# cyanreg/ffmpeg_ffv2

Hardware: AMD Instinct MI355X
Metric: Mpix/s encode (4K yuv420p10, slices=8) at 1/2/4/8 GPUs; bit-exact vs CPU (higher is better)
Workload: dtype int32

## Files before the change

### ffmpeg_ffv2_amd/csrc/ffv2_capi.cpp

```cpp
#include "../../include/ffv2_amd.h"
#include "ffv2_kernels.h"

#include <float.h>
#include <math.h>
#include <stdio.h>
#include <stdlib.h>
#include <string.h>

#include <atomic>
#include <chrono>
#include <condition_variable>
#include <functional>
#include <mutex>
#include <thread>
#include <vector>

#include "gen/scan_lut.h"

#define FFV2AMD_VERSION "ffv2-amd 0.1 (gfx950)"

namespace {

inline uint32_t coded_gain_host(int64_t e)
{
// ... 496 lines not shown
    }
    return FFV2AMD_ERR_INVAL;
}

size_t align_up(size_t v, size_t a) { return (v + a - 1) / a * a; }

}

struct ffv2amd_encoder;
static void lanecoder_free(ffv2amd_encoder *e);

struct ffv2amd_encoder {
    ffv2amd_info info{};
    FFV2Geom geom{};
    int device = 0;
    hipStream_t stream = nullptr;
    int64_t  *d_thr = nullptr;
    uint16_t *d_lds_scan = nullptr;
    uint8_t  *d_prefix = nullptr;
    int prefix_len = 0, slack = 0;
    uint32_t *d_codes = nullptr, *d_bitoff = nullptr;
    int32_t  *d_status = nullptr;
    int32_t  *d_err = nullptr;
    uint8_t  *d_frame = nullptr, *d_pkt = nullptr;
    uint32_t *d_meta = nullptr;
    int32_t  *d_w1 = nullptr;
    uint8_t  *h_frame = nullptr, *h_pkt = nullptr;
    uint32_t *h_meta = nullptr;
    int32_t *d_coef_ws = nullptr;
    int16_t *d_y = nullptr, *h_y = nullptr;
    uint32_t *h_codes = nullptr;
    uint8_t *d_pk_ws = nullptr;
    int32_t *d_inv_plane = nullptr;
    uint32_t *d_sizes_ws = nullptr;
    int32_t *coef_sink = nullptr;
    int profiling = 0;
    unsigned prof_calls = 0;
    struct EvTriple { hipEvent_t a, b, c, d; bool d_is_b; };
    bool pipelined = false;
    hipStream_t e_stream = nullptr;
    hipEvent_t evT[2] = { nullptr, nullptr }, evE[2] = { nullptr, nullptr };
    bool evE_valid[2] = { false, false };
    uint32_t *d_codes2 = nullptr, *d_bitoff2 = nullptr;
    int32_t *d_status2 = nullptr;
    unsigned seq = 0;
    int seq_pb = 0;
// ... 22 lines not shown
    bool device_coder = false;
    QpSet qset[2];
    size_t q_stream_stride = 0;
    hipStream_t q_copy = nullptr;
    unsigned q_sub = 0, q_fin = 0;
    uint8_t *qh_frame[2] = { nullptr, nullptr }, *qd_frame[2] = { nullptr, nullptr };
    int32_t *qd_w[2] = { nullptr, nullptr };
    uint8_t *qd_c420[2] = { nullptr, nullptr };
    int64_t q_tag[2] = { 0, 0 };
    int16_t *d_dec_pulses = nullptr;
    float *d_dec_mag = nullptr;
    int32_t *d_dec_c0 = nullptr, *d_dec_coef = nullptr;
    uint8_t *d_dec_frame = nullptr;
    int32_t *d_wide_plane = nullptr, *d_wide_c0 = nullptr;
    int64_t *d_wide_en = nullptr;
    FFV2Upconv *upconv = nullptr;
    bool upconv_tried = false;
    uint8_t *d_420 = nullptr, *h_420 = nullptr;
    struct RingSlot {
        uint8_t  *h_frame = nullptr, *d_frame = nullptr;
        uint8_t  *d_pkt = nullptr, *h_pkt = nullptr;
        uint32_t *d_meta = nullptr, *h_meta = nullptr;
        uint32_t *d_codes = nullptr, *d_bitcnt = nullptr;
        int32_t  *d_w = nullptr;
        bool has_w = false;
        uint8_t  *d_c420 = nullptr;
        hipEvent_t ev_h2d = nullptr, ev_done = nullptr, ev_meta = nullptr;
        int64_t tag = 0;
    };
    std::vector<RingSlot> ring;
    int ring_head = 0, ring_count = 0;
    hipStream_t ring_h2d = nullptr, ring_comp[2] = { nullptr, nullptr }, ring_d2h = nullptr, ring_pkt = nullptr;
    GatherPool *ring_pool = nullptr;
    unsigned ring_seq = 0;
    struct RegRange { const uint8_t *base; size_t bytes; };
    std::vector<RegRange> ring_reg;
    struct LaneCoder {
        int cap = 0;
        int group = 0;
        int32_t *d_coef = nullptr;
        int16_t *d_y = nullptr;
        uint32_t *d_bitcnt = nullptr;
        FFV2LaneCoderArgs a{};
        uint2 *d_split = nullptr;
        struct Set {
            uint32_t *d_codes = nullptr, *bits = nullptr, *rowbase = nullptr, *gbase = nullptr, *rawbase = nullptr, *delta = nullptr;
// ... 64 lines not shown

#define HIPCHK(x) do { hipError_t e_ = (x); if (e_ != hipSuccess) { \
    fprintf(stderr, "ffv2amd: %s failed: %s\n", #x, hipGetErrorString(e_)); \
    (void)hipGetLastError();       \
    return FFV2AMD_ERR_DEVICE; } } while (0)

struct DeviceGuard {
    int prev = -1;
    bool ok = false;
    explicit DeviceGuard(int dev)
    {
        if (hipGetDevice(&prev) != hipSuccess) prev = -1;
        ok = (prev == dev) || hipSetDevice(dev) == hipSuccess;
        if (prev == dev) prev = -1;
    }
    ~DeviceGuard() { if (prev >= 0) (void)hipSetDevice(prev); }
};

extern "C" void ffv2amd_ring_close(ffv2amd_encoder *e);
static int encode_uploaded_frame(ffv2amd_encoder *e, int qp, const int32_t *W, uint8_t *out, size_t out_cap, size_t *out_size);

static int launch_encode_qp0(ffv2amd_encoder *e, int nframes, const void *d_frames, const int32_t *d_W,
                             void *d_packets, size_t packet_stride, uint32_t *d_sizes, int32_t *status,
                             uint32_t *codes, uint32_t *bitcnt, int32_t *coef, hipStream_t st, hipStream_t se,
                             ffv2amd_encoder::EvTriple *ev, int32_t *err)
{
    FFV2TStageArgs a{};
    a.g = e->geom; a.nframes = nframes; a.frames = (const uint8_t *)d_frames;
    a.coef = coef; a.energy = nullptr; a.codes = codes; a.bitcnt = bitcnt; a.W = d_W;
    a.gain_thr = e->d_thr; a.gain_n = GAIN_TABLE_N; a.lds_scan = e->d_lds_scan;
    a.status = err;
    a.zero = (uint32_t *)d_packets; a.zero_stride_dw = (uint32_t)(packet_stride / 4);
    if (ev) HIPCHK(hipEventRecord(ev->a, st));
    HIPCHK(ffv2_launch_tstage(a, st));
    if (ev) HIPCHK(hipEventRecord(ev->b, st));
    if (se != st) {
        hipEvent_t join = e->evT[e->seq_pb];
        HIPCHK(hipEventRecord(join, st));
        HIPCHK(hipStreamWaitEvent(se, join, 0));
    }
    if (ev && se != st) HIPCHK(hipEventRecord(ev->d, se));
    if (ev) ev->d_is_b = se == st;
    FFV2EStageArgs b{};
    b.g = e->geom; b.nframes = nframes; b.codes = codes; b.bitoff = bitcnt;
    b.packets = (uint8_t *)d_packets; b.packet_stride = packet_stride;
    b.sizes = d_sizes; b.status = status; b.err = err;
    b.prefix = e->d_prefix; b.prefix_len = e->prefix_len; b.slack_bits = e->slack;
    b.header_bits = ((uint32_t)e->info.pix_fmt & 15u) | (1u << 4);
    b.header_nbits = 5;
    HIPCHK(ffv2_launch_estage_qp0(b, se));
    if (ev) HIPCHK(hipEventRecord(ev->c, se));
    return FFV2AMD_OK;
}

extern "C" {

const char *ffv2amd_version(void) { return FFV2AMD_VERSION; }

uint32_t ffv2amd_coded_gain(int64_t energy) { return coded_gain_host(energy); }

int ffv2amd_range_prefix(int pix_fmt, int num_sb, uint8_t *out, size_t cap, int *slack_bits)
{
    std::vector<uint8_t> b;
    int sl = 0;
    int r = range_prefix(pix_fmt, num_sb, b, &sl);
    if (r < 0) return r;
    if (b.size() > cap) return FFV2AMD_ERR_NOSPACE;
// ... 13 lines not shown
    (void)hipFree(e->d_420);
    if (e->h_420) (void)hipHostFree(e->h_420);
    lanecoder_free(e);
    for (auto &q : e->qset) {
        (void)hipFree(q.d_rec); (void)hipFree(q.d_stream); (void)hipFree(q.d_totals); (void)hipFree(q.d_codes); (void)hipFree(q.d_status);
        if (q.h_rec) (void)hipHostFree(q.h_rec);
        if (q.h_stream) (void)hipHostFree(q.h_stream);
        if (q.h_totals) (void)hipHostFree(q.h_totals);
        if (q.h_codes) (void)hipHostFree(q.h_codes);
        if (q.h_status) (void)hipHostFree(q.h_status);
        if (q.ev) (void)hipEventDestroy(q.ev);
        for (auto ev : q.ev_frame) if (ev) (void)hipEventDestroy(ev);
        (void)hipFree(q.d_pre); (void)hipFree(q.d_raw); (void)hipFree(q.d_pk); (void)hipFree(q.d_pk_sizes); (void)hipFree(q.d_pk_status);
        if (q.h_pk_sizes) (void)hipHostFree(q.h_pk_sizes);
        if (q.h_pk_status) (void)hipHostFree(q.h_pk_status);
    }
    if (e->q_copy) { (void)hipStreamSynchronize(e->q_copy); (void)hipStreamDestroy(e->q_copy); }
    for (int k = 0; k < 2; k++) {
        (void)hipFree(e->qd_frame[k]); (void)hipFree(e->qd_w[k]); (void)hipFree(e->qd_c420[k]);
        if (e->qh_frame[k]) (void)hipHostFree(e->qh_frame[k]);
    }
    (void)hipFree(e->d_thr); (void)hipFree(e->d_lds_scan); (void)hipFree(e->d_prefix);
    (void)hipFree(e->d_codes); (void)hipFree(e->d_bitoff); (void)hipFree(e->d_status); (void)hipFree(e->d_err);
    (void)hipFree(e->d_frame); (void)hipFree(e->d_pkt); (void)hipFree(e->d_meta); (void)hipFree(e->d_w1);
    (void)hipFree(e->d_inv_plane);
    (void)hipFree(e->d_wide_plane); (void)hipFree(e->d_wide_c0); (void)hipFree(e->d_wide_en);
    (void)hipFree(e->d_dec_pulses); (void)hipFree(e->d_dec_mag); (void)hipFree(e->d_dec_c0); (void)hipFree(e->d_dec_coef);
    (void)hipFree(e->d_dec_frame);
    (void)hipFree(e->d_coef_ws); (void)hipFree(e->d_y); (void)hipFree(e->d_pk_ws); (void)hipFree(e->d_sizes_ws);
    if (e->h_y) (void)hipHostFree(e->h_y);
    if (e->h_codes) (void)hipHostFree(e->h_codes);
    if (e->h_frame) (void)hipHostFree(e->h_frame);
    if (e->h_pkt) (void)hipHostFree(e->h_pkt);
    if (e->h_meta) (void)hipHostFree(e->h_meta);
    for (auto &t : e->ev_pool) { (void)hipEventDestroy(t.a); (void)hipEventDestroy(t.b); (void)hipEventDestroy(t.c); (void)hipEventDestroy(t.d); }
    if (e->e_stream) { (void)hipStreamSynchronize(e->e_stream); (void)hipStreamDestroy(e->e_stream); }
    for (int i = 0; i < 2; i++) { if (e->evT[i]) (void)hipEventDestroy(e->evT[i]); if (e->evE[i]) (void)hipEventDestroy(e->evE[i]); }
    (void)hipFree(e->d_codes2); (void)hipFree(e->d_bitoff2); (void)hipFree(e->d_status2);
    if (e->stream) (void)hipStreamDestroy(e->stream);
    (void)hipGetLastError();
    delete e;
}

int ffv2amd_encoder_create(ffv2amd_encoder **out, int width, int height, int pix_fmt,
                           int device, int max_batch)
{
// ... 41 lines not shown
    g.width = width; g.height = height; g.depth = depth; g.planes = planes; g.bytes_per_sample = bps;
    g.nsx = in.num_sb_x; g.nsy = in.num_sb_y; g.nblk = in.block_planes;
    g.row_pitch = in.row_pitch; g.plane_stride = in.plane_stride; g.frame_stride = in.frame_stride;
    g.inv_planes = (uint32_t)(((uint64_t)1 << 32) / (uint32_t)planes + 1);
    g.inv_nsx = (uint32_t)(((uint64_t)1 << 32) / (uint32_t)g.nsx + 1);

    std::call_once(g_thr_once, build_gain_table);
    uint16_t lds_scan[4096];
    for (int i = 0; i < 8; i++)
        for (int l = 0; l < 64; l++)
            for (int e = 0; e < 8; e++) {
                const int q = 256 * (2 * i + e / 4) + 4 * l + (e & 3);
                lds_scan[(i * 64 + l) * 8 + e] =
                    (uint16_t)(((FFV2_SCAN_LUT[q] >> 6) * 69 + (FFV2_SCAN_LUT[q] & 63)) * 4);
            }

#define CK(x) do { if ((x) != hipSuccess) { fprintf(stderr, "ffv2amd: %s failed: %s\n", #x, hipGetErrorString(hipGetLastError())); \
    ffv2amd_encoder_destroy(e); return FFV2AMD_ERR_DEVICE; } } while (0)
    CK(hipStreamCreateWithFlags(&e->stream, hipStreamNonBlocking));
    CK(hipMalloc(&e->d_thr, sizeof(int64_t) * GAIN_TABLE_N));
    CK(hipMemcpy(e->d_thr, g_thr.data(), sizeof(int64_t) * GAIN_TABLE_N, hipMemcpyHostToDevice));
    CK(hipMalloc(&e->d_lds_scan, sizeof(lds_scan)));
    CK(hipMemcpy(e->d_lds_scan, lds_scan, sizeof(lds_scan), hipMemcpyHostToDevice));
    CK(hipMalloc(&e->d_prefix, align_up(prefix.size(), 16)));
    CK(hipMemcpy(e->d_prefix, prefix.data(), prefix.size(), hipMemcpyHostToDevice));
    CK(hipMalloc(&e->d_codes, sizeof(uint32_t) * FFV2_CODES_PER_BP * g.nblk * (size_t)max_batch));
    CK(hipMalloc(&e->d_bitoff, sizeof(uint32_t) * g.nblk * (size_t)max_batch));
    CK(hipMalloc(&e->d_status, sizeof(int32_t) * (size_t)max_batch));
    CK(hipMalloc(&e->d_err, sizeof(int32_t) * 2 * (size_t)max_batch));
    CK(hipMemsetAsync(e->d_err, 0, sizeof(int32_t) * 2 * (size_t)max_batch, e->stream));
    CK(hipStreamSynchronize(e->stream));
    CK(hipStreamSynchronize(nullptr));
    CK(hipMalloc(&e->d_frame, in.frame_stride));
    CK(hipMalloc(&e->d_pkt, in.packet_cap));
    CK(hipMalloc(&e->d_meta, 16));
    CK(hipMalloc(&e->d_w1, sizeof(int32_t) * g.nblk));
    CK(hipHostMalloc(&e->h_frame, in.frame_stride, hipHostMallocDefault));
    CK(hipHostMalloc(&e->h_pkt, in.packet_cap, hipHostMallocDefault));
    CK(hipHostMalloc(&e->h_meta, 16, hipHostMallocDefault));
#undef CK
    memset(e->h_frame, 0, in.frame_stride);
    *out = e;
    return FFV2AMD_OK;
}

int ffv2amd_encoder_info(const ffv2amd_encoder *e, ffv2amd_info *info)
{
    if (!e || !info) return FFV2AMD_ERR_INVAL;
    *info = e->info;
    return FFV2AMD_OK;
}

int ffv2amd_tstage_device(ffv2amd_encoder *e, int nframes, const void *d_frames,
// ... 30 lines not shown
    const int pb = pipe ? (int)(e->seq++ & 1u) : 0;
    int32_t *status = d_status ? d_status : (pb ? e->d_status2 : e->d_status);
    uint32_t *codes = pb ? e->d_codes2 : e->d_codes, *bitcnt = pb ? e->d_bitoff2 : e->d_bitoff;
    hipStream_t se = pipe ? e->e_stream : s;
    if (pipe && e->evE_valid[pb])
        HIPCHK(hipStreamWaitEvent(s, e->evE[pb], 0));
    ffv2amd_encoder::EvTriple *ev = nullptr;
    if (e->profiling > 0 && (e->prof_calls++ % (unsigned)e->profiling) == 0) {
        if (e->ev_used == e->ev_pool.size()) {
            if (e->ev_pool.size() >= 8192) {
                double t, x, lo, hi; int n;
                ffv2amd_profile_read_ex(e, &t, &x, &n, &lo, &hi);
                e->prof_t = t; e->prof_e = x; e->prof_n = n; e->prof_tmin = lo; e->prof_tmax = hi;
            } else {
                ffv2amd_encoder::EvTriple t{};
                HIPCHK(hipEventCreate(&t.a)); HIPCHK(hipEventCreate(&t.b)); HIPCHK(hipEventCreate(&t.c));
                HIPCHK(hipEventCreate(&t.d));
                try { e->ev_pool.push_back(t); } catch (...) { return FFV2AMD_ERR_NOMEM; }
            }
        }
        ev = &e->ev_pool[e->ev_used++];
    }
    e->seq_pb = pb;
    int r = launch_encode_qp0(e, nframes, d_frames, d_W, d_packets, packet_stride, d_sizes, status, codes, bitcnt,
                              e->coef_sink, s, se, ev, e->d_err + (size_t)pb * e->info.max_batch);
    if (r < 0) return r;
    if (pipe) {
        HIPCHK(hipEventRecord(e->evE[pb], se));
        e->evE_valid[pb] = true;
    }
    return FFV2AMD_OK;
}

int ffv2amd_encoder_set_pipelined(ffv2amd_encoder *e, int on)
{
    if (!e) return FFV2AMD_ERR_INVAL;
    DeviceGuard guard(e->device);
    if (!guard.ok) return FFV2AMD_ERR_DEVICE;
    if (on && !e->e_stream) {
        const size_t nb = (size_t)e->info.block_planes, B = (size_t)e->info.max_batch;
        HIPCHK(hipStreamCreateWithFlags(&e->e_stream, hipStreamNonBlocking));
        for (int i = 0; i < 2; i++) {
            HIPCHK(hipEventCreateWithFlags(&e->evT[i], hipEventDisableTiming));
            HIPCHK(hipEventCreateWithFlags(&e->evE[i], hipEventDisableTiming));
        }
        HIPCHK(hipMalloc(&e->d_codes2, sizeof(uint32_t) * FFV2_CODES_PER_BP * nb * B));
        HIPCHK(hipMalloc(&e->d_bitoff2, sizeof(uint32_t) * nb * B));
        HIPCHK(hipMalloc(&e->d_status2, sizeof(int32_t) * B));
// ... 1518 lines not shown
                                     h_packets + (size_t)f * packet_stride, packet_stride, &n);
        } catch (...) { r = FFV2AMD_ERR_NOMEM; }
        h_status[f] = r;
        h_sizes[f] = r < 0 ? 0 : (uint32_t)n;
    });
    if (trace) {
        const auto t_end = std::chrono::steady_clock::now();
        fprintf(stderr, "ffv2amd: qp=%d batch of %d: device (T-stage + PVQ + copies) %.3f ms, host range coder %.3f ms\n",
                qp, nframes, std::chrono::duration<double, std::milli>(t_dev - t_begin).count(),
                std::chrono::duration<double, std::milli>(t_end - t_dev).count());
    }
    return FFV2AMD_OK;
}


void ffv2amd_ring_close(ffv2amd_encoder *e)
{
    if (!e || e->ring.empty()) return;
    (void)hipSetDevice(e->device);
    for (hipStream_t st : { e->ring_h2d, e->ring_comp[0], e->ring_comp[1], e->ring_d2h, e->ring_pkt })
        if (st) (void)hipStreamSynchronize(st);
    for (auto &r : e->ring) {
        (void)hipFree(r.d_frame); (void)hipFree(r.d_pkt); (void)hipFree(r.d_meta);
        (void)hipFree(r.d_codes); (void)hipFree(r.d_bitcnt); (void)hipFree(r.d_w); (void)hipFree(r.d_c420);
        if (r.h_frame) (void)hipHostFree(r.h_frame);
        if (r.h_pkt) (void)hipHostFree(r.h_pkt);
        if (r.h_meta) (void)hipHostFree(r.h_meta);
        if (r.ev_h2d) (void)hipEventDestroy(r.ev_h2d);
        if (r.ev_done) (void)hipEventDestroy(r.ev_done);
        if (r.ev_meta) (void)hipEventDestroy(r.ev_meta);
    }
    e->ring.clear();
    for (auto &g : e->ring_reg) (void)hipHostUnregister((void *)g.base);
    e->ring_reg.clear();
    if (e->ring_pool) { e->ring_pool->shutdown(); delete e->ring_pool; e->ring_pool = nullptr; }
    for (hipStream_t *st : { &e->ring_h2d, &e->ring_comp[0], &e->ring_comp[1], &e->ring_d2h, &e->ring_pkt })
        if (*st) { (void)hipStreamDestroy(*st); *st = nullptr; }
    e->ring_head = e->ring_count = 0;
}

int ffv2amd_ring_open(ffv2amd_encoder *e, int depth)
{
    if (!e || depth < 1 || depth > 64) return FFV2AMD_ERR_INVAL;
    if (!e->ring.empty()) return FFV2AMD_ERR_INVAL;
    DeviceGuard guard(e->device);
    if (!guard.ok) return FFV2AMD_ERR_DEVICE;
    const ffv2amd_info &in = e->info;
    const size_t nb = (size_t)in.block_planes;
#define RK(x) do { if ((x) != hipSuccess) { fprintf(stderr, "ffv2amd: %s failed: %s\n", #x, hipGetErrorString(hipGetLastError())); \
    ffv2amd_ring_close(e); return FFV2AMD_ERR_DEVICE; } } while (0)
    try { e->ring.resize((size_t)depth); } catch (...) { return FFV2AMD_ERR_NOMEM; }
    RK(hipStreamCreateWithFlags(&e->ring_h2d, hipStreamNonBlocking));
    RK(hipStreamCreateWithFlags(&e->ring_comp[0], hipStreamNonBlocking));
    RK(hipStreamCreateWithFlags(&e->ring_comp[1], hipStreamNonBlocking));
    RK(hipStreamCreateWithFlags(&e->ring_d2h, hipStreamNonBlocking));
    RK(hipStreamCreateWithFlags(&e->ring_pkt, hipStreamNonBlocking));
    for (auto &r : e->ring) {
        RK(hipMalloc(&r.d_frame, in.frame_stride));
        RK(hipMalloc(&r.d_pkt, in.packet_cap));
        RK(hipMalloc(&r.d_meta, 16));
        RK(hipMemsetAsync(r.d_meta, 0, 16, e->ring_d2h));
        RK(hipMalloc(&r.d_codes, sizeof(uint32_t) * FFV2_CODES_PER_BP * nb));
        RK(hipMalloc(&r.d_bitcnt, sizeof(uint32_t) * nb));
        RK(hipMalloc(&r.d_w, sizeof(int32_t) * nb));
        RK(hipHostMalloc(&r.h_frame, in.frame_stride, hipHostMallocDefault));
        RK(hipHostMalloc(&r.h_pkt, in.packet_cap, hipHostMallocDefault));
        RK(hipHostMalloc(&r.h_meta, 16, hipHostMallocDefault));
        RK(hipEventCreateWithFlags(&r.ev_h2d, hipEventDisableTiming));
        RK(hipEventCreateWithFlags(&r.ev_done, hipEventDisableTiming));
        RK(hipEventCreateWithFlags(&r.ev_meta, hipEventDisableTiming));
    }
    RK(hipStreamSynchronize(e->ring_d2h));
#undef RK
    e->ring_head = e->ring_count = 0;
    if (e->info.frame_stride >= ((size_t)8 << 20)) {
        unsigned hw = std::thread::hardware_concurrency();
        static const int want = getenv("FFV2AMD_GATHER_THREADS") ? atoi(getenv("FFV2AMD_GATHER_THREADS")) : 6;
        const int helpers = (int)hw >= want ? want - 1 : (hw > 1 ? (int)hw - 1 : 0);
        e->ring_pool = new (std::nothrow) GatherPool;
        if (e->ring_pool && helpers > 0) e->ring_pool->start(helpers, e->device);
    }
    return FFV2AMD_OK;
}

int ffv2amd_ring_pending(const ffv2amd_encoder *e) { return e ? e->ring_count : 0; }

// ... 70 lines not shown
            up[i] = hipMemcpyAsync(q.d_dst + (size_t)y0 * q.pitch, q.stage + (size_t)y0 * q.pitch, (size_t)(y1 - y0) * q.pitch,
                                   hipMemcpyHostToDevice, sh);
        };
        if (e->ring_pool) {
            try { e->ring_pool->run(nsl, slice); } catch (...) { return FFV2AMD_ERR_NOMEM; }
        } else {
            for (int i = 0; i < nsl; i++) slice(i);
        }
        for (int i = 0; i < nsl; i++) HIPCHK(up[i]);
    }
    const int32_t *dW = nullptr;
    r.has_w = W != nullptr;
    if (W) {
        HIPCHK(hipMemcpyAsync(r.d_w, W, sizeof(int32_t) * in.block_planes, hipMemcpyHostToDevice, sh));
        dW = r.d_w;
    }
    HIPCHK(hipEventRecord(r.ev_h2d, sh));
    hipStream_t sc = e->ring_comp[e->ring_seq++ & 1u];
    HIPCHK(hipStreamWaitEvent(sc, r.ev_h2d, 0));
    if (chroma420)
        HIPCHK(ffv2_launch_upconv_chroma(e->upconv, e->geom, 1, r.d_c420, pl[1].pitch, pl[1].pitch * (size_t)pl[1].rows, 0,
                                         r.d_frame, sc));
    int rc = launch_encode_qp0(e, 1, r.d_frame, dW, r.d_pkt, in.packet_cap, r.d_meta, (int32_t *)(r.d_meta + 1),
                               r.d_codes, r.d_bitcnt, nullptr, sc, sc, nullptr, (int32_t *)(r.d_meta + 2));
    if (rc < 0) return rc;
    HIPCHK(hipEventRecord(r.ev_done, sc));
    HIPCHK(hipStreamWaitEvent(e->ring_d2h, r.ev_done, 0));
    HIPCHK(hipMemcpyAsync(r.h_meta, r.d_meta, 8, hipMemcpyDeviceToHost, e->ring_d2h));
    HIPCHK(hipEventRecord(r.ev_meta, e->ring_d2h));
    r.tag = tag;
    e->ring_count++;
    return FFV2AMD_OK;
}

int ffv2amd_ring_send(ffv2amd_encoder *e, const uint8_t *const data[4], const ptrdiff_t linesize[4],
                      const int32_t *W, int64_t tag, unsigned flags)
{
    if (!e || !data || !linesize || e->ring.empty()) return FFV2AMD_ERR_INVAL;
    const ffv2amd_info &in = e->info;
    for (int p = 0; p < in.planes; p++)
        if (!data[p]) return FFV2AMD_ERR_INVAL;
    if (e->ring_count == (int)e->ring.size()) return FFV2AMD_ERR_AGAIN;
    DeviceGuard guard(e->device);
    if (!guard.ok) return FFV2AMD_ERR_DEVICE;
    auto &r = e->ring[(size_t)((e->ring_head + e->ring_count) % (int)e->ring.size())];
    RingPlane pl[4];
    for (int p = 0; p < in.planes; p++)
// ... 74 lines not shown
```

### ffmpeg_ffv2_amd/csrc/ffv2_kernels.h

```cpp
#pragma once
#include <hip/hip_runtime.h>
#include <stdint.h>

#define FFV2_NUM_BANDS     13
#define FFV2_CODES_PER_BP  16

struct FFV2Geom {
    int width, height, depth, planes, bytes_per_sample;
    int nsx, nsy, nblk;
    size_t row_pitch, plane_stride, frame_stride;
    uint32_t inv_planes, inv_nsx;
};

struct FFV2TStageArgs {
    FFV2Geom g;
    int nframes;
    const uint8_t *frames;
    int32_t  *coef;
    int64_t  *energy;
    uint32_t *codes;
    uint32_t *bitcnt;
    const int32_t *W;
    const int64_t *gain_thr;
    int gain_n;
    const uint16_t *lds_scan;
    int32_t *status;
    uint32_t *zero;
    uint32_t zero_stride_dw;
};

struct FFV2EStageArgs {
    FFV2Geom g;
    int nframes;
    const uint32_t *codes;
    const uint32_t *bitoff;
    uint8_t  *packets;
    size_t    packet_stride;
    uint32_t *sizes;
    int32_t  *status;
    int32_t  *err;
    const uint8_t *prefix;
    int prefix_len, slack_bits;
    uint32_t header_bits, header_nbits;
};

#define FFV2_Y_STRIDE 4104

hipError_t ffv2_launch_tstage(const FFV2TStageArgs &a, hipStream_t s);
void ffv2_tstage_force_variant(int mode);
const char *ffv2_tstage_kernel_name(const FFV2Geom &g, int nframes, bool coef_writeback);
hipError_t ffv2_launch_inverse(const FFV2Geom &g, int nframes, const int32_t *coef, int32_t *plane,
                               uint8_t *frames, const uint16_t *lds_scan, hipStream_t s);
hipError_t ffv2_launch_dequant(const int16_t *pulses, const float *mag, const int32_t *c0, int32_t *coef, long long nbp,
                               hipStream_t s);
struct FFV2SymRec {
    uint32_t offset;
    uint16_t count[FFV2_NUM_BANDS];
    uint16_t pad;
// ... 79 lines not shown
```

### ffmpeg_ffv2_amd/csrc/ffv2_kernels.hip

```cpp
#include "ffv2_kernels.h"

#include "gen/fdct64_net.h"
#ifdef FFV2_ASM_NET
#include "gen/fdct64_asm.h"
#endif

#include <stdio.h>
#include <stdlib.h>

#define FFV2_WALK_MIN 2

__device__ __forceinline__ int ffv2_rsh1(int a)
{
    int t;
    asm("v_sub_u32_sdwa %0, %1, sext(%1) dst_sel:DWORD dst_unused:UNUSED_PAD src0_sel:DWORD src1_sel:BYTE_3"
        : "=v"(t) : "v"(a));
    return t >> 1;
}
#define FFV2_RSH1(a)            ffv2_rsh1(a)
#define FFV2_MULRS_WRAP(a, K, R, S)  ((__mul24((a), (K)) + (R)) >> (S))
#define FFV2_MULRS_NOOVF(a, K, R, S) (((K) < (1 << ((S) - 1))) \
    ? (int)(((long long)(a) * (int)((long long)(K) << (32 - (S))) + 0x80000000LL) >> 32) \
    : FFV2_MULRS_WRAP(a, K, R, S))

// ... 257 lines not shown
        a.energy[((size_t)f * g.nblk + bp) * FFV2_NUM_BANDS + band] = (long long)my;

    if (a.codes) {
        if (band == 12 && has_band && a.W) {
            const long long w = a.W[(size_t)f * g.nblk + bp];
            my += (unsigned long long)(w * w);
        }
        bool oot = false;
        uint32_t val = 0;
        int nb = 0;
        if (has_band) {
            val = coded_gain((long long)my, a.gain_thr, a.gain_n, oot);
            nb = golomb_len(val);
        } else if (lane == 0) {
            const int c0 = x[0];
            val = (uint32_t)c0;
            const uint32_t mag = c0 < 0 ? (uint32_t)(-(long long)c0) : (uint32_t)c0;
            nb = golomb_len(mag) + (c0 != 0);
        }
        nb = wave_iscan(nb);
        uint32_t *rec = a.codes + ((size_t)f * g.nblk + bp) * FFV2_CODES_PER_BP;
        if (has_band)        rec[1 + band] = val;
        else if (lane == 0)  rec[0] = val;
        else if (lane == 63) { rec[14] = (uint32_t)nb; a.bitcnt[(size_t)f * g.nblk + bp] = (uint32_t)nb; }
        else if (lane == 1)  rec[15] = 0;
        if (__any(oot) && lane == 0)
            atomicMin(&a.status[f], -34);
    }
    if (WRITE_COEF) {
        typedef int i32x4 __attribute__((ext_vector_type(4)));
        i32x4 *cp = reinterpret_cast<i32x4 *>(a.coef + ((size_t)f * g.nblk + bp) * 4096);
#pragma unroll
        for (int j = 0; j < 16; j++) {
            const i32x4 v = { x[4 * j], x[4 * j + 1], x[4 * j + 2], x[4 * j + 3] };
            __builtin_nontemporal_store(v, &cp[j * 64 + lane]);
        }
    }
    if (a.zero) {
        const uint32_t per = (a.zero_stride_dw + (uint32_t)g.nblk - 1u) / (uint32_t)g.nblk;
        uint32_t *z = a.zero + (size_t)f * a.zero_stride_dw;
        for (uint32_t d = (uint32_t)lane; d < per; d += 64) {
            const uint32_t i = (uint32_t)bp * per + d;
            if (i < a.zero_stride_dw) z[i] = 0;
        }
    }
}

// ... 482 lines not shown
#pragma unroll
            for (int it = 0; it < PL_MAIN; it++)
                asm("" : "=v"(v[it].x), "=v"(v[it].y), "=v"(v[it].z), "=v"(v[it].w));
        }
        uint4 lut[8];
        WALK_MARK(0);
        tstage_back_half<WRITE_COEF, true>(x, lut, xb, a, f, bp, lane, lane_info);
        WALK_MARK(1);
#ifdef FFV2_PHASE_TIMING
        wdone_++;
#endif
    }
#ifdef FFV2_PHASE_TIMING
    if (lane == 0) {
        unsigned long long *pt_ = g_phase_buf + (size_t)blockIdx.x * 8;
        pt_[0] = wrt0_; pt_[1] = __builtin_amdgcn_s_getreg((4 << 0) | (0 << 6) | (31 << 11));
        pt_[2] = __builtin_amdgcn_s_memrealtime() - wrt0_;
        pt_[3] = wacc_[0]; pt_[4] = wacc_[1]; pt_[5] = wacc_[2]; pt_[6] = wdone_;
    }
#endif
}


constexpr int EP_THREADS = 256;
constexpr int EP_WORDS   = 3840;

struct LdsBitSink {
    uint32_t *buf;
    uint32_t word;
    unsigned long long win;
    int nwin;
    __device__ void init(uint32_t *b, uint32_t bitpos)
    {
        buf = b; word = bitpos >> 5; nwin = (int)(bitpos & 31); win = 0;
    }
    __device__ void put(unsigned long long v, int n)
    {
        win |= v << nwin;
        nwin += n;
        if (nwin >= 32) {
            atomicOr(&buf[word++], (uint32_t)win);
            win >>= 32;
            nwin -= 32;
        }
    }
    __device__ void flush()
    {
        if (nwin > 0 && (uint32_t)win) atomicOr(&buf[word], (uint32_t)win);
// ... 13 lines not shown

__device__ __forceinline__ void put_golomb(LdsBitSink &s, uint32_t val)
{
    const uint32_t v = val + 1;
    const int nb = 31 - __clz(v);
    unsigned long long pat = 1ull << (2 * nb);
    if (nb > 0) {
        const uint32_t m = v & ((1u << nb) - 1);
        const uint32_t r = __brev(m) >> (32 - nb);
        pat |= spread_bits(r) << 1;
    }
    const int len = 2 * nb + 1;
    if (len > 32) {
        s.put(pat & 0xffffffffull, 32);
        s.put(pat >> 32, len - 32);
    } else {
        s.put(pat, len);
    }
}

__global__ __launch_bounds__(EP_THREADS) void ffv2_estage_kernel(const FFV2EStageArgs a)
{
    __shared__ uint32_t bits[EP_WORDS];
    __shared__ uint32_t scratch[8];
    const int f = blockIdx.y, tid = threadIdx.x;
    const int n = a.g.nblk, P = a.g.planes;
    const int i0 = blockIdx.x * EP_THREADS;
    const uint32_t *cnt = a.bitoff + (size_t)f * n;
    const int i = i0 + tid;
    const bool have = i < n;
    uint4 r0 = make_uint4(0, 0, 0, 0), r1 = r0, r2 = r0, r3 = r0;
    if (have) {
        const uint4 *rp = reinterpret_cast<const uint4 *>(a.codes + ((size_t)f * n + i) * FFV2_CODES_PER_BP);
        r0 = rp[0]; r1 = rp[1]; r2 = rp[2]; r3 = rp[3];
    }

    uint32_t before = 0, all = 0;
    for (int i = tid; i < n; i += EP_THREADS) {
        const uint32_t v = cnt[i];
        all += v;
        before += i < i0 ? v : 0u;
    }
    {
        const uint32_t b = (uint32_t)__builtin_amdgcn_readlane(wave_iscan((int)before), 63);
        const uint32_t t = (uint32_t)__builtin_amdgcn_readlane(wave_iscan((int)all), 63);
        if ((tid & 63) == 0) { scratch[tid >> 6] = b; scratch[4 + (tid >> 6)] = t; }
        __syncthreads();
        before = scratch[0] + scratch[1] + scratch[2] + scratch[3] + 4u * (uint32_t)((i0 + P - 1) / P);
        all = scratch[4] + scratch[5] + scratch[6] + scratch[7] + 4u * (uint32_t)(n / P);
    }

    const uint32_t tx = (have && (i % P) == 0) ? 4u : 0u;
    const uint32_t mine = have ? r3.z + tx : 0u;
    const uint32_t incl = (uint32_t)wave_iscan((int)mine);
    __syncthreads();
    if ((tid & 63) == 63) scratch[tid >> 6] = incl;
    __syncthreads();
    uint32_t wbase = 0;
    for (int w = 0; w < (tid >> 6); w++) wbase += scratch[w];
    const uint32_t local_total = scratch[0] + scratch[1] + scratch[2] + scratch[3];

    const uint32_t total_bits = a.header_nbits + all;
    const uint32_t slack = (uint32_t)a.slack_bits;
    const uint32_t nraw = total_bits > slack ? (total_bits - slack + 7) >> 3 : 0;
    const uint32_t total = (uint32_t)a.prefix_len + nraw;
    uint8_t *pkt = a.packets + (size_t)f * a.packet_stride;
    const bool fits = (size_t)total + 4 <= a.packet_stride;
    if (blockIdx.x == 0 && tid == 0) {
        a.sizes[f] = fits ? total : 0;
        int32_t st = a.err[f];
        a.err[f] = 0;
        if (!fits && st > -28) st = -28;
        a.status[f] = st;
    }
    if (!fits) return;

    const uint32_t B0 = blockIdx.x == 0 ? 0u : a.header_nbits + before;
    const uint32_t B1 = a.header_nbits + before + local_total;
    const uint32_t lbase = B0 & ~31u;
    const uint32_t nwords = (B1 - lbase + 31) >> 5;
    for (uint32_t w = tid; w < nwords + 1 && w < EP_WORDS; w += EP_THREADS) bits[w] = 0;
    __syncthreads();

    if (have) {
        const uint32_t rec[14] = { r0.x, r0.y, r0.z, r0.w, r1.x, r1.y, r1.z, r1.w,
                                   r2.x, r2.y, r2.z, r2.w, r3.x, r3.y };
        LdsBitSink s;
        s.init(bits, a.header_nbits + before + wbase + (incl - mine) + tx - lbase);
        const int c0 = (int)rec[0];
        const uint32_t mag = c0 < 0 ? (uint32_t)(-(long long)c0) : (uint32_t)c0;
        put_golomb(s, mag);
        if (c0) s.put(c0 < 0 ? 1u : 0u, 1);
#pragma unroll
        for (int b = 0; b < FFV2_NUM_BANDS; b++)
            put_golomb(s, rec[1 + b]);
        s.flush();
    }
    if (blockIdx.x == 0 && tid == 0)
        atomicOr(&bits[0], a.header_bits);
    __syncthreads();

    const uint32_t ka = B0 >> 3, kb = (B1 + 7) >> 3;
    const uint32_t ea = (B0 + 7) >> 3, eb = B1 >> 3;
    if (kb > ka) {
        const uint32_t dlo = (total - kb) & ~3u, dhi = (total - 1 - ka) & ~3u;
        const uint8_t *lb = reinterpret_cast<const uint8_t *>(bits);
        for (uint32_t d = dlo + 4 * tid; d <= dhi; d += 4 * EP_THREADS) {
            uint32_t word = 0;
            bool exclusive = true;
#pragma unroll
            for (int j = 0; j < 4; j++) {
                const int64_t k = (int64_t)total - 1 - (int64_t)(d + j);
                const bool ours = k >= (int64_t)ka && k < (int64_t)kb;
                exclusive = exclusive && k >= (int64_t)ea && k < (int64_t)eb;
                const uint32_t v = ours ? lb[(uint32_t)k - (lbase >> 3)] : 0u;
                word |= v << (8 * j);
            }
            uint32_t *dst = reinterpret_cast<uint32_t *>(pkt + d);
            if (exclusive) *dst = word;
            else if (word) atomicOr(dst, word);
        }
    }
    if (blockIdx.x == 0)
        for (int k = tid; k < a.prefix_len; k += EP_THREADS)
            atomicOr(reinterpret_cast<uint32_t *>(pkt + (k & ~3)), (uint32_t)a.prefix[k] << ((k & 3) * 8));
}

}

static int walk_slots(bool bps2, bool wc)
{
    static int cache[16][4];
    int dev = 0;
    if (hipGetDevice(&dev) != hipSuccess || dev < 0 || dev >= 16) return 0;
    int &c = cache[dev][(bps2 ? 2 : 0) + (wc ? 1 : 0)];
    if (c == 0) {
        int per_cu = 0, cus = 0;
        const void *fn = bps2 ? (wc ? (const void *)ffv2_tstage_walk_kernel<2, true> : (const void *)ffv2_tstage_walk_kernel<2, false>)
                              : (wc ? (const void *)ffv2_tstage_walk_kernel<1, true> : (const void *)ffv2_tstage_walk_kernel<1, false>);
        if (hipOccupancyMaxActiveBlocksPerMultiprocessor(&per_cu, fn, 64, 0) != hipSuccess ||
            hipDeviceGetAttribute(&cus, hipDeviceAttributeMultiprocessorCount, dev) != hipSuccess || per_cu < 1 || cus < 1)
            c = -1;
        else
            c = per_cu * cus;
    }
    return c;
}

// ... 72 lines not shown
```

Before: 180,200.

## Replace estage global bit-count scan with per-chunk totals accumulated in tstage

The transform stage now atomically adds each block-plane's bit count into per-chunk totals (64 block-planes per chunk). The entropy stage becomes one wave per chunk: it sums the short chunk-total array to get its prefix offset instead of rescanning every bitcnt entry, and it drops the LDS scratch and block-wide syncs. The last arriving wave resets the totals through an arrival counter. This trades a per-block O(n) reduction for more, smaller blocks plus global atomics and self-cleaning state, which adds ordering risk across frames and buffers.

```diff
diff --git a/ffmpeg_ffv2_amd/csrc/ffv2_capi.cpp b/ffmpeg_ffv2_amd/csrc/ffv2_capi.cpp
--- a/ffmpeg_ffv2_amd/csrc/ffv2_capi.cpp
+++ b/ffmpeg_ffv2_amd/csrc/ffv2_capi.cpp
@@ -542,6 +542,7 @@
     uint32_t *d_codes = nullptr, *d_bitoff = nullptr;
     int32_t  *d_status = nullptr;
     int32_t  *d_err = nullptr;
+    uint32_t *d_chunks = nullptr;
     uint8_t  *d_frame = nullptr, *d_pkt = nullptr;
     uint32_t *d_meta = nullptr;
     int32_t  *d_w1 = nullptr;
@@ -610,6 +611,7 @@
         uint8_t  *d_pkt = nullptr, *h_pkt = nullptr;
         uint32_t *d_meta = nullptr, *h_meta = nullptr;
         uint32_t *d_codes = nullptr, *d_bitcnt = nullptr;
+        uint32_t *d_chunks = nullptr;
         int32_t  *d_w = nullptr;
         bool has_w = false;
         uint8_t  *d_c420 = nullptr;
@@ -720,12 +722,14 @@
 
 static int launch_encode_qp0(ffv2amd_encoder *e, int nframes, const void *d_frames, const int32_t *d_W,
                              void *d_packets, size_t packet_stride, uint32_t *d_sizes, int32_t *status,
-                             uint32_t *codes, uint32_t *bitcnt, int32_t *coef, hipStream_t st, hipStream_t se,
-                             ffv2amd_encoder::EvTriple *ev, int32_t *err)
-{
+                             uint32_t *codes, uint32_t *bitcnt, uint32_t *chunks, int32_t *coef, hipStream_t st,
+                             hipStream_t se, ffv2amd_encoder::EvTriple *ev, int32_t *err)
+{
+    const uint32_t cstride = ffv2_chunk_stride(e->geom.nblk);
     FFV2TStageArgs a{};
     a.g = e->geom; a.nframes = nframes; a.frames = (const uint8_t *)d_frames;
     a.coef = coef; a.energy = nullptr; a.codes = codes; a.bitcnt = bitcnt; a.W = d_W;
+    a.chunk_bits = chunks; a.chunk_stride = cstride;
     a.gain_thr = e->d_thr; a.gain_n = GAIN_TABLE_N; a.lds_scan = e->d_lds_scan;
     a.status = err;
     a.zero = (uint32_t *)d_packets; a.zero_stride_dw = (uint32_t)(packet_stride / 4);
@@ -740,7 +744,7 @@
     if (ev && se != st) HIPCHK(hipEventRecord(ev->d, se));
     if (ev) ev->d_is_b = se == st;
     FFV2EStageArgs b{};
-    b.g = e->geom; b.nframes = nframes; b.codes = codes; b.bitoff = bitcnt;
+    b.g = e->geom; b.nframes = nframes; b.codes = codes; b.chunk_bits = chunks; b.chunk_stride = cstride;
     b.packets = (uint8_t *)d_packets; b.packet_stride = packet_stride;
     b.sizes = d_sizes; b.status = status; b.err = err;
     b.prefix = e->d_prefix; b.prefix_len = e->prefix_len; b.slack_bits = e->slack;
@@ -800,6 +804,7 @@
     }
     (void)hipFree(e->d_thr); (void)hipFree(e->d_lds_scan); (void)hipFree(e->d_prefix);
     (void)hipFree(e->d_codes); (void)hipFree(e->d_bitoff); (void)hipFree(e->d_status); (void)hipFree(e->d_err);
+    (void)hipFree(e->d_chunks);
     (void)hipFree(e->d_frame); (void)hipFree(e->d_pkt); (void)hipFree(e->d_meta); (void)hipFree(e->d_w1);
     (void)hipFree(e->d_inv_plane);
     (void)hipFree(e->d_wide_plane); (void)hipFree(e->d_wide_c0); (void)hipFree(e->d_wide_en);
@@ -887,13 +892,16 @@
     CK(hipMemcpy(e->d_thr, g_thr.data(), sizeof(int64_t) * GAIN_TABLE_N, hipMemcpyHostToDevice));
     CK(hipMalloc(&e->d_lds_scan, sizeof(lds_scan)));
     CK(hipMemcpy(e->d_lds_scan, lds_scan, sizeof(lds_scan), hipMemcpyHostToDevice));
-    CK(hipMalloc(&e->d_prefix, align_up(prefix.size(), 16)));
+    CK(hipMalloc(&e->d_prefix, align_up(prefix.size() + 1, 16)));
     CK(hipMemcpy(e->d_prefix, prefix.data(), prefix.size(), hipMemcpyHostToDevice));
     CK(hipMalloc(&e->d_codes, sizeof(uint32_t) * FFV2_CODES_PER_BP * g.nblk * (size_t)max_batch));
     CK(hipMalloc(&e->d_bitoff, sizeof(uint32_t) * g.nblk * (size_t)max_batch));
     CK(hipMalloc(&e->d_status, sizeof(int32_t) * (size_t)max_batch));
     CK(hipMalloc(&e->d_err, sizeof(int32_t) * 2 * (size_t)max_batch));
+    const size_t chunk_bytes = sizeof(uint32_t) * ffv2_chunk_stride(g.nblk) * 2 * (size_t)max_batch;
+    CK(hipMalloc(&e->d_chunks, chunk_bytes));
     CK(hipMemsetAsync(e->d_err, 0, sizeof(int32_t) * 2 * (size_t)max_batch, e->stream));
+    CK(hipMemsetAsync(e->d_chunks, 0, chunk_bytes, e->stream));
     CK(hipStreamSynchronize(e->stream));
     CK(hipStreamSynchronize(nullptr));
     CK(hipMalloc(&e->d_frame, in.frame_stride));
@@ -970,8 +978,9 @@
         ev = &e->ev_pool[e->ev_used++];
     }
     e->seq_pb = pb;
+    uint32_t *chunks = e->d_chunks + (size_t)pb * e->info.max_batch * ffv2_chunk_stride(e->geom.nblk);
     int r = launch_encode_qp0(e, nframes, d_frames, d_W, d_packets, packet_stride, d_sizes, status, codes, bitcnt,
-                              e->coef_sink, s, se, ev, e->d_err + (size_t)pb * e->info.max_batch);
+                              chunks, e->coef_sink, s, se, ev, e->d_err + (size_t)pb * e->info.max_batch);
     if (r < 0) return r;
     if (pipe) {
         HIPCHK(hipEventRecord(e->evE[pb], se));
@@ -2536,7 +2545,7 @@
         if (st) (void)hipStreamSynchronize(st);
     for (auto &r : e->ring) {
         (void)hipFree(r.d_frame); (void)hipFree(r.d_pkt); (void)hipFree(r.d_meta);
-        (void)hipFree(r.d_codes); (void)hipFree(r.d_bitcnt); (void)hipFree(r.d_w); (void)hipFree(r.d_c420);
+        (void)hipFree(r.d_codes); (void)hipFree(r.d_bitcnt); (void)hipFree(r.d_chunks); (void)hipFree(r.d_w); (void)hipFree(r.d_c420);
         if (r.h_frame) (void)hipHostFree(r.h_frame);
         if (r.h_pkt) (void)hipHostFree(r.h_pkt);
         if (r.h_meta) (void)hipHostFree(r.h_meta);
@@ -2576,6 +2585,8 @@
         RK(hipMemsetAsync(r.d_meta, 0, 16, e->ring_d2h));
         RK(hipMalloc(&r.d_codes, sizeof(uint32_t) * FFV2_CODES_PER_BP * nb));
         RK(hipMalloc(&r.d_bitcnt, sizeof(uint32_t) * nb));
+        RK(hipMalloc(&r.d_chunks, sizeof(uint32_t) * ffv2_chunk_stride(in.block_planes)));
+        RK(hipMemsetAsync(r.d_chunks, 0, sizeof(uint32_t) * ffv2_chunk_stride(in.block_planes), e->ring_d2h));
         RK(hipMalloc(&r.d_w, sizeof(int32_t) * nb));
         RK(hipHostMalloc(&r.h_frame, in.frame_stride, hipHostMallocDefault));
         RK(hipHostMalloc(&r.h_pkt, in.packet_cap, hipHostMallocDefault));
@@ -2692,7 +2703,7 @@
         HIPCHK(ffv2_launch_upconv_chroma(e->upconv, e->geom, 1, r.d_c420, pl[1].pitch, pl[1].pitch * (size_t)pl[1].rows, 0,
                                          r.d_frame, sc));
     int rc = launch_encode_qp0(e, 1, r.d_frame, dW, r.d_pkt, in.packet_cap, r.d_meta, (int32_t *)(r.d_meta + 1),
-                               r.d_codes, r.d_bitcnt, nullptr, sc, sc, nullptr, (int32_t *)(r.d_meta + 2));
+                               r.d_codes, r.d_bitcnt, r.d_chunks, nullptr, sc, sc, nullptr, (int32_t *)(r.d_meta + 2));
     if (rc < 0) return rc;
     HIPCHK(hipEventRecord(r.ev_done, sc));
     HIPCHK(hipStreamWaitEvent(e->ring_d2h, r.ev_done, 0));
diff --git a/ffmpeg_ffv2_amd/csrc/ffv2_kernels.h b/ffmpeg_ffv2_amd/csrc/ffv2_kernels.h
--- a/ffmpeg_ffv2_amd/csrc/ffv2_kernels.h
+++ b/ffmpeg_ffv2_amd/csrc/ffv2_kernels.h
@@ -12,6 +12,10 @@
     uint32_t inv_planes, inv_nsx;
 };
 
+#define FFV2_EP_CHUNK 64
+static inline uint32_t ffv2_chunk_span(int nblk) { return (uint32_t)((nblk + 64 * 128 - 1) / (64 * 128)) * 128u; }
+static inline uint32_t ffv2_chunk_stride(int nblk) { return ffv2_chunk_span(nblk) + 32u; }
+
 struct FFV2TStageArgs {
     FFV2Geom g;
     int nframes;
@@ -20,6 +24,8 @@
     int64_t  *energy;
     uint32_t *codes;
     uint32_t *bitcnt;
+    uint32_t *chunk_bits;
+    uint32_t chunk_stride;
     const int32_t *W;
     const int64_t *gain_thr;
     int gain_n;
@@ -33,7 +39,8 @@
     FFV2Geom g;
     int nframes;
     const uint32_t *codes;
-    const uint32_t *bitoff;
+    uint32_t *chunk_bits;
+    uint32_t chunk_stride;
     uint8_t  *packets;
     size_t    packet_stride;
     uint32_t *sizes;
diff --git a/ffmpeg_ffv2_amd/csrc/ffv2_kernels.hip b/ffmpeg_ffv2_amd/csrc/ffv2_kernels.hip
--- a/ffmpeg_ffv2_amd/csrc/ffv2_kernels.hip
+++ b/ffmpeg_ffv2_amd/csrc/ffv2_kernels.hip
@@ -303,7 +303,11 @@
         uint32_t *rec = a.codes + ((size_t)f * g.nblk + bp) * FFV2_CODES_PER_BP;
         if (has_band)        rec[1 + band] = val;
         else if (lane == 0)  rec[0] = val;
-        else if (lane == 63) { rec[14] = (uint32_t)nb; a.bitcnt[(size_t)f * g.nblk + bp] = (uint32_t)nb; }
+        else if (lane == 63) {
+            rec[14] = (uint32_t)nb; a.bitcnt[(size_t)f * g.nblk + bp] = (uint32_t)nb;
+            if (a.chunk_bits)
+                atomicAdd(&a.chunk_bits[(size_t)f * a.chunk_stride + (uint32_t)bp / FFV2_EP_CHUNK], (uint32_t)nb);
+        }
         else if (lane == 1)  rec[15] = 0;
         if (__any(oot) && lane == 0)
             atomicMin(&a.status[f], -34);
@@ -832,8 +836,8 @@
 }
 
 
-constexpr int EP_THREADS = 256;
-constexpr int EP_WORDS   = 3840;
+constexpr int EP_THREADS = FFV2_EP_CHUNK;
+constexpr int EP_WORDS   = 960;
 
 struct LdsBitSink {
     uint32_t *buf;
@@ -893,43 +897,54 @@
 __global__ __launch_bounds__(EP_THREADS) void ffv2_estage_kernel(const FFV2EStageArgs a)
 {
     __shared__ uint32_t bits[EP_WORDS];
-    __shared__ uint32_t scratch[8];
-    const int f = blockIdx.y, tid = threadIdx.x;
+    const int f = blockIdx.y, lane = threadIdx.x;
     const int n = a.g.nblk, P = a.g.planes;
-    const int i0 = blockIdx.x * EP_THREADS;
-    const uint32_t *cnt = a.bitoff + (size_t)f * n;
-    const int i = i0 + tid;
+    const uint32_t c = blockIdx.x, nch = gridDim.x;
+    const int i0 = (int)c * EP_THREADS;
+    uint32_t *tot = a.chunk_bits + (size_t)f * a.chunk_stride;
+    const uint32_t span = a.chunk_stride - 32u;
+    const int i = i0 + lane;
     const bool have = i < n;
-    uint4 r0 = make_uint4(0, 0, 0, 0), r1 = r0, r2 = r0, r3 = r0;
-    if (have) {
-        const uint4 *rp = reinterpret_cast<const uint4 *>(a.codes + ((size_t)f * n + i) * FFV2_CODES_PER_BP);
-        r0 = rp[0]; r1 = rp[1]; r2 = rp[2]; r3 = rp[3];
-    }
+    const uint4 *rp = reinterpret_cast<const uint4 *>(a.codes + ((size_t)f * n + (have ? i : n - 1)) * FFV2_CODES_PER_BP);
+    const uint4 r0 = rp[0], r1 = rp[1], r2 = rp[2], r3 = rp[3];
+    const int pwn = (a.prefix_len + 3) >> 2;
+    const uint32_t *pw = reinterpret_cast<const uint32_t *>(a.prefix);
+    const uint32_t pre = pw[lane < pwn ? lane : 0];
+    const int32_t err = a.err[f];
 
     uint32_t before = 0, all = 0;
-    for (int i = tid; i < n; i += EP_THREADS) {
-        const uint32_t v = cnt[i];
-        all += v;
-        before += i < i0 ? v : 0u;
-    }
-    {
-        const uint32_t b = (uint32_t)__builtin_amdgcn_readlane(wave_iscan((int)before), 63);
-        const uint32_t t = (uint32_t)__builtin_amdgcn_readlane(wave_iscan((int)all), 63);
-        if ((tid & 63) == 0) { scratch[tid >> 6] = b; scratch[4 + (tid >> 6)] = t; }
-        __syncthreads();
-        before = scratch[0] + scratch[1] + scratch[2] + scratch[3] + 4u * (uint32_t)((i0 + P - 1) / P);
-        all = scratch[4] + scratch[5] + scratch[6] + scratch[7] + 4u * (uint32_t)(n / P);
-    }
+    for (uint32_t j = (uint32_t)lane; j < span; j += 2 * EP_THREADS) {
+        const uint32_t v0 = tot[j], v1 = tot[j + EP_THREADS];
+        all += v0 + v1;
+        before += (j < c ? v0 : 0u) + (j + EP_THREADS < c ? v1 : 0u);
+    }
+    asm volatile("s_waitcnt vmcnt(0)" :: "v"(r0.x), "v"(r0.y), "v"(r0.z), "v"(r0.w), "v"(r1.x), "v"(r1.y), "v"(r1.z),
+                 "v"(r1.w), "v"(r2.x), "v"(r2.y), "v"(r2.z), "v"(r2.w), "v"(r3.x), "v"(r3.y), "v"(r3.z), "v"(r3.w),
+                 "v"(pre), "v"(err) : "memory");
+    uint32_t opaque0;
+    asm volatile("v_mov_b32 %0, 0" : "=v"(opaque0));
+    uint32_t arrived = 0;
+    if (lane == 0) arrived = atomicAdd(&tot[span + opaque0], 1u);
+    before = (uint32_t)__builtin_amdgcn_readlane(wave_iscan((int)before), 63) + 4u * (uint32_t)((i0 + P - 1) / P);
+    all = (uint32_t)__builtin_amdgcn_readlane(wave_iscan((int)all), 63) + 4u * (uint32_t)(n / P);
 
     const uint32_t tx = (have && (i % P) == 0) ? 4u : 0u;
     const uint32_t mine = have ? r3.z + tx : 0u;
     const uint32_t incl = (uint32_t)wave_iscan((int)mine);
-    __syncthreads();
-    if ((tid & 63) == 63) scratch[tid >> 6] = incl;
-    __syncthreads();
-    uint32_t wbase = 0;
-    for (int w = 0; w < (tid >> 6); w++) wbase += scratch[w];
-    const uint32_t local_total = scratch[0] + scratch[1] + scratch[2] + scratch[3];
+    const uint32_t local_total = (uint32_t)__builtin_amdgcn_readlane((int)incl, 63);
+
+    auto retire = [&](const bool fits) {
+        if (c == 0 && lane == 0) {
+            int32_t st = err;
+            a.err[f] = 0;
+            if (!fits && st > -28) st = -28;
+            a.status[f] = st;
+        }
+        if ((uint32_t)__builtin_amdgcn_readlane((int)arrived, 0) == nch - 1u) {
+            for (uint32_t j = (uint32_t)lane; j < nch; j += EP_THREADS) tot[j] = 0;
+            if (lane == 0) __hip_atomic_store(&tot[span], 0u, __ATOMIC_RELAXED, __HIP_MEMORY_SCOPE_AGENT);
+        }
+    };
 
     const uint32_t total_bits = a.header_nbits + all;
     const uint32_t slack = (uint32_t)a.slack_bits;
@@ -937,27 +952,24 @@
     const uint32_t total = (uint32_t)a.prefix_len + nraw;
     uint8_t *pkt = a.packets + (size_t)f * a.packet_stride;
     const bool fits = (size_t)total + 4 <= a.packet_stride;
-    if (blockIdx.x == 0 && tid == 0) {
-        a.sizes[f] = fits ? total : 0;
-        int32_t st = a.err[f];
-        a.err[f] = 0;
-        if (!fits && st > -28) st = -28;
-        a.status[f] = st;
-    }
-    if (!fits) return;
-
-    const uint32_t B0 = blockIdx.x == 0 ? 0u : a.header_nbits + before;
+    if (c == 0 && lane == 0) a.sizes[f] = fits ? total : 0;
+    if (!fits) {
+        retire(false);
+        return;
+    }
+
+    const uint32_t B0 = c == 0 ? 0u : a.header_nbits + before;
     const uint32_t B1 = a.header_nbits + before + local_total;
     const uint32_t lbase = B0 & ~31u;
     const uint32_t nwords = (B1 - lbase + 31) >> 5;
-    for (uint32_t w = tid; w < nwords + 1 && w < EP_WORDS; w += EP_THREADS) bits[w] = 0;
+    for (uint32_t w = lane; w < nwords + 1 && w < EP_WORDS; w += EP_THREADS) bits[w] = 0;
     __syncthreads();
 
     if (have) {
         const uint32_t rec[14] = { r0.x, r0.y, r0.z, r0.w, r1.x, r1.y, r1.z, r1.w,
                                    r2.x, r2.y, r2.z, r2.w, r3.x, r3.y };
         LdsBitSink s;
-        s.init(bits, a.header_nbits + before + wbase + (incl - mine) + tx - lbase);
+        s.init(bits, a.header_nbits + before + (incl - mine) + tx - lbase);
         const int c0 = (int)rec[0];
         const uint32_t mag = c0 < 0 ? (uint32_t)(-(long long)c0) : (uint32_t)c0;
         put_golomb(s, mag);
@@ -967,7 +979,7 @@
             put_golomb(s, rec[1 + b]);
         s.flush();
     }
-    if (blockIdx.x == 0 && tid == 0)
+    if (c == 0 && lane == 0)
         atomicOr(&bits[0], a.header_bits);
     __syncthreads();
 
@@ -976,7 +988,7 @@
     if (kb > ka) {
         const uint32_t dlo = (total - kb) & ~3u, dhi = (total - 1 - ka) & ~3u;
         const uint8_t *lb = reinterpret_cast<const uint8_t *>(bits);
-        for (uint32_t d = dlo + 4 * tid; d <= dhi; d += 4 * EP_THREADS) {
+        for (uint32_t d = dlo + 4 * lane; d <= dhi; d += 4 * EP_THREADS) {
             uint32_t word = 0;
             bool exclusive = true;
 #pragma unroll
@@ -992,9 +1004,15 @@
             else if (word) atomicOr(dst, word);
         }
     }
-    if (blockIdx.x == 0)
-        for (int k = tid; k < a.prefix_len; k += EP_THREADS)
-            atomicOr(reinterpret_cast<uint32_t *>(pkt + (k & ~3)), (uint32_t)a.prefix[k] << ((k & 3) * 8));
+    if (c == 0) {
+        for (int w = lane; w < pwn; w += EP_THREADS) {
+            const uint32_t word = w < EP_THREADS ? pre : pw[w];
+            const int nb = a.prefix_len - 4 * w;
+            const uint32_t v = nb >= 4 ? word : word & ((1u << (8 * nb)) - 1u);
+            if (v) atomicOr(reinterpret_cast<uint32_t *>(pkt + 4 * w), v);
+        }
+    }
+    retire(true);
 }
 
 }
```

Result: no change. 179,200 (median of 6 runs) (-0.6%).
